# daac-tools/daachorse

Hardware: NVIDIA H100
Metric: input GB/s scanned, find_overlapping_iter, 675k-pat bytewise (higher is better)
Workload: dtype u8

## Files before the change

daachorse_b200/csrc/dev_image.cpp:

```cpp
#include "dev_image.h"

#include <algorithm>

namespace dach {

namespace {

bool fail_chains_terminate(const dach_pma* p, bool dead_is_terminal) {
    const size_t n = p->slots();
    std::vector<uint8_t> color(n, 0);
    std::vector<uint32_t> path;
    for (size_t start = 0; start < n; ++start) {
        if (color[start]) continue;
        path.clear();
        uint32_t s = uint32_t(start);
        for (;;) {
            if (s == kRoot || (dead_is_terminal && s == kDead) || color[s] == 2) break;
            if (color[s] == 1) return false;
            color[s] = 1;
            path.push_back(s);
            s = p->fail[s];
        }
        for (uint32_t v : path) color[v] = 2;
    }
// ... 148 lines not shown
            used[found ^ c] = 1;
            R->new_of_old[b_old ^ c] = found ^ c;
            moved[b_old ^ c] = 1;
            --n_free;
        }
    }
    for (size_t s = 0; s < n; ++s) {
        if (s != kRoot && s != kDead && !moved[s]) R->new_of_old[s] = uint32_t(s) + H;
        if (!rebased[s] && p->base[s] != 0) R->new_base[s] = p->base[s] + H;
    }
    R->vacant_check.assign(H, 0);
    for (uint32_t blk = 0; blk < H; blk += 256) {
        uint32_t ub = blk == 0 ? 0u : kNone;
        for (uint32_t b = blk; ub == kNone && b < blk + 256; ++b)
            if (!base_used[b]) {
                ub = b;
                break;
            }
        for (uint32_t v = blk; v < blk + 256; ++v)
            if (!used[v] || v == kRoot || v == kDead) R->vacant_check[v] = ub == kNone ? 0x100u : (0x100u | ((ub ^ v) & 0xffu));
    }
    R->hot_slots = H;
}

}

int build_image(const dach_pma* p, HostImage* img) {
    const size_t n = p->slots();
    const bool lm = is_leftmost(p->match_kind);
    img->charwise = p->charwise;
    img->match_kind = p->match_kind;
    img->n_slots = uint32_t(n);
    img->root_opos = n ? p->state_output_pos(kRoot) : 0;
    img->max_pattern_len = 0;
    for (const OutputRec& o : p->outputs)
        if (o.length > img->max_pattern_len) img->max_pattern_len = o.length;

    if (n >= 0x80000000ull) {
        set_error("automaton too large for the device image (2^31 slots)");
        return DACH_AUTOMATON_SCALE;
    }
    if (!fail_chains_terminate(p, p->charwise || lm)) {
        set_error("invalid automaton: a failure chain never reaches the root");
        return DACH_INVALID_AUTOMATON;
    }

    img->outputs.resize(p->outputs.size() * 4);
    for (size_t i = 0; i < p->outputs.size(); ++i) {
        img->outputs[i * 4 + 0] = p->outputs[i].value;
        img->outputs[i * 4 + 1] = p->outputs[i].length;
        img->outputs[i * 4 + 2] = p->outputs[i].parent;
        const uint32_t par = p->outputs[i].parent;
        img->outputs[i * 4 + 3] = 1u + (par ? img->outputs[(size_t)(par - 1) * 4 + 3] : 0u);
    }

    img->rec.resize(n * 4);
    if (!p->charwise) {
        auto skip_leaves = [&](uint32_t f) {
            while (f != kRoot && !(lm && f == kDead) && p->base[f] == 0) f = p->fail[f];
            return f;
        };
        for (size_t s = 0; s < n; ++s) {
            const uint32_t f = skip_leaves(p->fail[s]);
            const bool terminal = f == kRoot || (lm && f == kDead);
            uint32_t* r = &img->rec[s * 4];
            r[0] = p->base[s];
            r[1] = f;
            r[2] = terminal ? 0 : p->base[f];
            if (!terminal && !lm && skip_leaves(p->fail[f]) == kRoot) r[2] |= 0x80000000u;
            r[3] = p->opos_ch[s];
        }
        img->root_table.assign(256, kRoot);
        if (n && p->base[kRoot] != 0) {
            const uint32_t b = p->base[kRoot];
            for (uint32_t c = 0; c < 256; ++c) {
                const uint32_t ci = b ^ c;
                if (ci < n && (p->opos_ch[ci] & 0xff) == c) img->root_table[c] = ci;
            }
        }
        img->root_base = n ? p->base[kRoot] : 0;
        img->hot_slots = 0;
        if (n <= (size_t(1) << 24) && p->outputs.size() < (size_t(1) << 24)) {
            Relayout R;
            relayout_bytewise(p, img->want_hot_slots, &R);
            img->segmentable = R.textbook && R.max_depth <= img->max_pattern_len;
            const uint32_t H = R.hot_slots;
            const size_t N = n + H;
            img->hot_slots = H;
            img->n_cslots = uint32_t(N);
            img->crec.assign(N * 4, 0);
            img->opos_tab.assign(N, 0);
            img->new_of_old = R.new_of_old;
            img->old_of_new.assign(N, kRoot);
            img->root_base = n ? R.new_base[kRoot] : 0;
            auto nid = [&](uint32_t s) { return s < n ? R.new_of_old[s] : s; };
            for (size_t s = 0; s < n; ++s) {
                const uint32_t* w = &img->rec[s * 4];
                const uint32_t ns = R.new_of_old[s];
                img->old_of_new[ns] = uint32_t(s);
                uint32_t* r = &img->crec[size_t(ns) * 4];
                const uint32_t opos = p->opos_ch[s] >> 8;
                const uint32_t f = w[1];
                const bool terminal = f == kRoot || (lm && f == kDead);
                uint32_t flags = opos ? 1u : 0u;
                uint32_t fbase = terminal ? 0u : R.new_base[f];
                if (!lm) {
// ... 71 lines not shown
```

daachorse_b200/csrc/dev_image.h:

```cpp
#pragma once

#include <cstdint>
#include <vector>

#include "host.h"

namespace dach {

struct HostImage {
    bool charwise = false;
    uint8_t match_kind = 0;
    uint32_t n_slots = 0;
    uint32_t root_opos = 0;
    uint32_t max_pattern_len = 0;
    std::vector<uint32_t> rec;
    std::vector<uint32_t> outputs;
    std::vector<uint32_t> root_table;
    std::vector<uint32_t> crec;
    std::vector<uint32_t> opos_tab;
    uint32_t root_base = 0;
    uint32_t want_hot_slots = 65536;
    uint32_t hot_slots = 0;
    uint32_t n_cslots = 0;
    std::vector<uint32_t> new_of_old;
    std::vector<uint32_t> old_of_new;
    std::vector<uint32_t> mapper;
    bool segmentable = false;
};

int build_image(const dach_pma* p, HostImage* img);

}
```

daachorse_b200/csrc/dev_scan.cu:

```cuda
#include <cuda_runtime.h>

#include <unistd.h>

#include <algorithm>
#include <atomic>
#include <chrono>
#include <cstdio>
#include <cstdlib>
#include <cstring>
#include <memory>
#include <mutex>
#include <string>
#include <vector>

#include "dev_image.h"
#include "host.h"
#include "scan_lane.cuh"

namespace dach {


constexpr int kMaxThreads = 1024;
constexpr int kMaxDevices = 64;
constexpr uint32_t kRootBytes = 1024;
// ... 502 lines not shown
                                                 const uint4* outputs, const uint32_t* opos_tab) {
    if (ctrl->overflow) return;
    const unsigned long long b0m = base ? *base : 0ull;
    if (b0m + item_offs[n_items] > out_cap) return;
    out_words += b0m * 3ull;
    if (pad_like) out_words += (*pad_like * 3ull) & 3ull;
    const uint32_t used = min(ctrl->blk_cursor, pool_blocks);
    const uint32_t lane = threadIdx.x & 31;
    const uint64_t warp = (uint64_t)blockIdx.x * (blockDim.x >> 5) + (threadIdx.x >> 5);
    const uint64_t n_warps = (uint64_t)gridDim.x * (blockDim.x >> 5);
    for (uint64_t b0 = warp * U; b0 < used; b0 += n_warps * U) {
        uint4 h[U], o[U];
        uint2 ev[U];
        uint32_t len[U];
#pragma unroll
        for (int u = 0; u < U; ++u) {
            const uint64_t b = b0 + u < used ? b0 + u : b0;
            const uint32_t* blk = pool + (blkmap ? (uint64_t)blkmap[b] : b) * BLK_WORDS;
            h[u] = *reinterpret_cast<const uint4*>(blk);
            ev[u] = lane < BLK_EVENTS ? reinterpret_cast<const uint2*>(blk + BLK_HDR_WORDS)[lane] : make_uint2(0u, 0u);
        }
#pragma unroll
        for (int u = 0; u < U; ++u) {
            const uint32_t nev = min(BLK_EVENTS, ev_counts[h[u].x] - h[u].y * BLK_EVENTS);
            const bool on = b0 + u < used && lane < nev;
            const uint32_t op = on ? ld_u32(opos_tab + (ev[u].y & QSLOT_MASK)) : 0u;
            o[u] = on ? ld_u4(outputs + (op - 1)) : make_uint4(0u, 0u, 0u, 0u);
            len[u] = on ? (OVERLAP ? o[u].w : 1u) : 0u;
        }
#pragma unroll
        for (int u = 0; u < U; ++u) {
            uint32_t inc = len[u];
#pragma unroll
            for (int d = 1; d < 32; d <<= 1) {
                const uint32_t t = __shfl_up_sync(0xffffffffu, inc, d);
                if (lane >= (uint32_t)d) inc += t;
            }
            if (!len[u]) continue;
            uint32_t* dst = out_words + (item_offs[h[u].x] + h[u].z + (inc - len[u])) * 3ull;
            const uint32_t end = ev[u].x;
            uint4 r = o[u];
            for (uint32_t k = 0;;) {
                dst[0] = end - r.y;
                dst[1] = end;
                dst[2] = r.x;
                if (++k == len[u]) break;
                dst += 3;
                r = ld_u4(outputs + (r.z - 1));
            }
        }
    }
}

__global__ void __launch_bounds__(128, 10) k_push(const uint32_t* src, const unsigned long long* total_ptr, const unsigned long long* base,
                                               unsigned long long out_cap, const ScanCtrl* ctrl, uint32_t* out_words) {
    if (ctrl->overflow) return;
    const unsigned long long b0 = base ? *base : 0ull, total = *total_ptr;
    if (b0 + total > out_cap) return;
    uint32_t* dst = out_words + b0 * 3ull;
    src += (b0 * 3ull) & 3ull;
    const unsigned long long n_words = total * 3ull;
    const unsigned long long head = min((unsigned long long)((4u - (uint32_t)(((uintptr_t)dst >> 2) & 3u)) & 3u), n_words);
    const unsigned long long n_vec = (n_words - head) / 4ull;
    const unsigned long long tid = (unsigned long long)blockIdx.x * blockDim.x + threadIdx.x;
    const unsigned long long nth = (unsigned long long)gridDim.x * blockDim.x;
    const uint4* s4 = reinterpret_cast<const uint4*>(src + head);
    uint4* d4 = reinterpret_cast<uint4*>(dst + head);
    unsigned long long v = tid;
#pragma unroll 1
    for (; v + 3ull * nth < n_vec; v += 4ull * nth) {
        const uint4 a = s4[v], b = s4[v + nth], c = s4[v + 2ull * nth], e = s4[v + 3ull * nth];
        d4[v] = a;
        d4[v + nth] = b;
        d4[v + 2ull * nth] = c;
        d4[v + 3ull * nth] = e;
    }
#pragma unroll 1
    for (; v < n_vec; v += nth) d4[v] = s4[v];
    const unsigned long long tail0 = head + 4ull * n_vec;
    if (tid < head) dst[tid] = src[tid];
    if (tid < n_words - tail0) dst[tail0 + tid] = src[tail0 + tid];
}

__global__ void __launch_bounds__(256) k_final_offsets(const unsigned long long* seg_first, const unsigned long long* item_offs,
                                                        uint64_t n, const unsigned long long* base, int last,
                                                        unsigned long long* out_offs, const ScanCtrl* ctrl) {
    if (ctrl->bad_offsets) return;
    const uint64_t h = (uint64_t)blockIdx.x * blockDim.x + threadIdx.x;
    if (h < n || (h == n && last)) out_offs[h] = (base ? *base : 0ull) + item_offs[seg_first ? seg_first[h] : h];
}

__global__ void __launch_bounds__(256) k_add_base(const ScanCtrl* ctrl, const unsigned long long* out_offs, uint64_t n,
                                                   unsigned long long out_cap, const uint32_t* pos_in, uint32_t* out_words) {
    if (ctrl->overflow || ctrl->bad_offsets) return;
    const unsigned long long total = out_offs[n];
    if (total > out_cap) return;
    for (unsigned long long m = (unsigned long long)blockIdx.x * blockDim.x + threadIdx.x; m < total;
         m += (unsigned long long)gridDim.x * blockDim.x) {
        uint64_t lo = 0, hi = n;
        while (lo + 1 < hi) {
            const uint64_t mid = (lo + hi) / 2;
            if (out_offs[mid] <= m)
                lo = mid;
            else
                hi = mid;
        }
// ... 231 lines not shown
        red_add_u64(df_acc + (uint32_t)keys.keys[keys.list[i]], 1);
}

__global__ void __launch_bounds__(256) k_df_clear(DfSet a, DfSet b) {
    const unsigned int na = *a.n, nb = *b.n;
    for (unsigned int i = blockIdx.x * blockDim.x + threadIdx.x; i < na; i += gridDim.x * blockDim.x) a.keys[a.list[i]] = DF_EMPTY;
    for (unsigned int i = blockIdx.x * blockDim.x + threadIdx.x; i < nb; i += gridDim.x * blockDim.x) b.keys[b.list[i]] = DF_EMPTY;
}

__global__ void __launch_bounds__(256) k_df_commit(const unsigned long long* acc, unsigned long long* df, uint64_t n) {
    for (uint64_t i = blockIdx.x * (uint64_t)blockDim.x + threadIdx.x; i < n; i += (uint64_t)gridDim.x * blockDim.x) df[i] += acc[i];
}

}


using namespace dach;

namespace {

struct DevBuf {
    void* p = nullptr;
    size_t bytes = 0;
};

bool cuda_ok(cudaError_t e, const char* what) {
    if (e == cudaSuccess) return true;
    set_error(std::string(what) + ": " + cudaGetErrorString(e));
    return false;
}

bool ensure(DevBuf& b, size_t bytes) {
    if (b.bytes >= bytes && b.p) return true;
    if (b.p) cudaFree(b.p);
    b.p = nullptr;
    b.bytes = 0;
    const size_t want = std::max<size_t>(bytes, 256);
    if (!cuda_ok(cudaMalloc(&b.p, want), "cudaMalloc")) return false;
    b.bytes = want;
    return true;
}

struct HostPinned {
    unsigned long long total;
    ScanCtrl ctrl;
    unsigned long long tail_offs[2];
    unsigned long long total_rk;
};

struct Workspace {
    DevBuf counts, ev_counts, tiles, ctrl, pool;
    DevBuf nseg, seg_first, item_hay, item_beg, item_offs, n_items_dev;
    DevBuf blk_first, blkmap, tiles2;
    DevBuf stage;
    DevBuf items_rk, total_rk;
    DevBuf slot_hist, rec_hist, hist_acc;
    HostPinned* pinned = nullptr;
    cudaEvent_t ev[4] = {nullptr, nullptr, nullptr, nullptr};
    cudaEvent_t ev_scanned = nullptr, ev_placed = nullptr;
    cudaEvent_t ev_push[2] = {nullptr, nullptr};
    uint64_t job_n = 0, job_items = 0;
    uint32_t job_pool_blocks = 0;
    uint64_t job_cap = 0;
    bool job_seg = false, job_ordered = false, job_open = false, job_placed = false;
    bool job_events = false;
    bool refused = false;
    int job_mode = 0;
    cudaStream_t job_stream = nullptr;
    DevBuf text, offs, out, out_offs;
    void* offs_stage = nullptr;
    size_t offs_stage_bytes = 0;
    cudaStream_t stream = nullptr;
    bool init(bool with_stream) {
        if (!pinned && !cuda_ok(cudaMallocHost(reinterpret_cast<void**>(&pinned), sizeof(HostPinned)), "cudaMallocHost"))
            return false;
        for (int i = 0; i < 4; ++i)
            if (!ev[i] && !cuda_ok(cudaEventCreate(&ev[i]), "cudaEventCreate")) return false;
        if (!ev_scanned && !cuda_ok(cudaEventCreateWithFlags(&ev_scanned, cudaEventDisableTiming), "cudaEventCreate")) return false;
        if (!ev_placed && !cuda_ok(cudaEventCreateWithFlags(&ev_placed, cudaEventDisableTiming), "cudaEventCreate")) return false;
        for (int i = 0; i < 2; ++i)
            if (!ev_push[i] && !cuda_ok(cudaEventCreate(&ev_push[i]), "cudaEventCreate")) return false;
        if (with_stream && !stream && !cuda_ok(cudaStreamCreateWithFlags(&stream, cudaStreamNonBlocking), "cudaStreamCreate"))
            return false;
        return true;
    }
    void release() {
        for (DevBuf* b : {&counts, &ev_counts, &tiles, &ctrl, &pool, &text, &offs, &out, &out_offs, &nseg, &seg_first, &item_hay, &item_beg,
                          &item_offs, &n_items_dev, &blk_first, &blkmap, &tiles2, &stage, &items_rk, &total_rk, &slot_hist, &rec_hist,
                          &hist_acc})
            if (b->p) {
                cudaFree(b->p);
                b->p = nullptr;
                b->bytes = 0;
            }
        if (pinned) cudaFreeHost(pinned);
        pinned = nullptr;
        if (offs_stage) cudaFreeHost(offs_stage);
        offs_stage = nullptr;
        offs_stage_bytes = 0;
        for (int i = 0; i < 4; ++i)
            if (ev[i]) {
                cudaEventDestroy(ev[i]);
                ev[i] = nullptr;
            }
        for (int i = 0; i < 2; ++i)
            if (ev_push[i]) {
                cudaEventDestroy(ev_push[i]);
                ev_push[i] = nullptr;
            }
        if (ev_scanned) cudaEventDestroy(ev_scanned);
        if (ev_placed) cudaEventDestroy(ev_placed);
        ev_scanned = ev_placed = nullptr;
        if (stream) cudaStreamDestroy(stream);
        stream = nullptr;
    }
};

}

struct dach_dev {
    int device = 0;
    bool charwise = false;
    uint8_t match_kind = 0;
    uint32_t n_slots = 0, root_opos = 0, mapper_len = 0, max_pattern_len = 0;
    bool segmentable = false;
    uint32_t n_outputs = 0, max_value = 0, n_cslots = 0;
    size_t image_bytes = 0;
    int sm_count = 0;
    size_t smem_optin = 0;
    uint4* d_rec = nullptr;
    uint4* d_outputs = nullptr;
    uint32_t* d_root = nullptr;
    uint4* d_crec = nullptr;
    uint32_t* d_opos = nullptr;
    uint32_t* d_id_in = nullptr;
    uint32_t* d_id_out = nullptr;
    uint32_t hot_slots = 0;
    uint32_t root_base = 0;
    uint32_t* d_mapper = nullptr;
    void* image_base = nullptr;
    size_t image_alloc = 0;
    std::mutex mu;
    Workspace ws;
    static constexpr int kSlots = 4;
    Workspace slot[kSlots];
    int64_t opt_slice_mib = 64;
    int64_t opt_hot_entries = kHotAuto;
    int64_t opt_event_queue = 0;
    int64_t opt_hist_smem = 1024;
    int64_t opt_df_pairs = kDefaultDfPairs;
    int64_t opt_slice_ramp = 1;
    int64_t opt_tail_seg = 0;
    int64_t opt_gather_ordered = 1;
    int64_t opt_gather_u = 4;
    int64_t opt_reserve_sms = 0;
    int64_t opt_smem_pad_kib = 0;
    int64_t opt_seg_len = 0;
    int64_t opt_hot_records = 0;
    int64_t opt_threads = 1024;
    int64_t opt_ctas_per_sm = 1;
    int64_t opt_l2_hints = 2;
    int64_t opt_kernel = 3;
    std::atomic<uint64_t> launches{0};
    cudaEvent_t ev_ref = nullptr;
    double last_scan_ms = 0, last_total_ms = 0;
    uint64_t last_h2d = 0, last_d2h = 0;
    DevBuf df_tab[2], df_list[2], df_n, df_acc;
    uint32_t df_mask = 0, df_limit = 0;
    bool df_clean = false;
    uint64_t last_df_windows = 0, last_df_rescans = 0;
    std::atomic<int> refs{1};
};

struct dach_job {
    dach_dev* d = nullptr;
    Workspace W;
    uint64_t out_cap = ~0ull;
};

namespace {

struct DeviceGuard {
    int prev = -1;
    bool ok = false;
    explicit DeviceGuard(int dev) {
        if (cudaGetDevice(&prev) != cudaSuccess) prev = -1;
        ok = cuda_ok(cudaSetDevice(dev), "cudaSetDevice");
        if (!ok) cudaGetLastError();
    }
    ~DeviceGuard() {
        if (prev >= 0) cudaSetDevice(prev);
    }
};

template <bool CW, int MODE>
cudaError_t launch_scan_t(const ScanParams& P, int grid, int threads, size_t smem, cudaStream_t st) {
    static bool attr_done[kMaxDevices] = {};
    int dev = 0;
    cudaGetDevice(&dev);
    if (dev < 0 || dev >= kMaxDevices || !attr_done[dev]) {
        cudaError_t e = cudaFuncSetAttribute(k_scan<CW, MODE>, cudaFuncAttributeMaxDynamicSharedMemorySize, 226 * 1024);
// ... 275 lines not shown
            want &= ~uint64_t(255);
        }
        smem = (size_t)want * 16 + queues;
        if (d->opt_smem_pad_kib > 0) smem = std::min<size_t>(smem + ((size_t)d->opt_smem_pad_kib << 10), smem_budget);
        P.hot_n = 0;
        P.hot_entries = (uint32_t)want;
    } else {
        uint64_t hot = smem_budget > kRootBytes ? (smem_budget - kRootBytes) / 16 : 0;
        if (d->opt_hot_records >= 0) hot = std::min<uint64_t>(hot, (uint64_t)d->opt_hot_records);
        hot = std::min<uint64_t>(hot, d->n_slots);
        P.hot_n = (uint32_t)hot;
        smem = kRootBytes + (size_t)hot * 16;
    }
    return smem;
}

void enqueue_seg_table(dach_dev* d, Workspace& W, const uint64_t* d_offs, uint64_t n, uint32_t seg_len, uint32_t seg_from,
                       ScanParams& P, cudaStream_t st) {
    unsigned long long* tiles = static_cast<unsigned long long*>(W.tiles.p);
    unsigned long long* seg_first = static_cast<unsigned long long*>(W.seg_first.p);
    const unsigned hb = (unsigned)((n + 255) / 256), hb1 = (unsigned)((n + 1 + 255) / 256);
    const uint64_t nt = (n + kScanTile - 1) / kScanTile;
    uint32_t* nseg = static_cast<uint32_t*>(W.nseg.p);
    k_seg_count<<<hb, 256, 0, st>>>(d_offs, n, seg_len, seg_from, nseg, P.ctrl);
    k_offsets_tile_sums<1><<<(unsigned)nt, kScanThreads, 0, st>>>(nseg, n, tiles);
    k_offsets_scan_tiles<<<1, kScanThreads, 0, st>>>(tiles, nt);
    k_offsets_apply<1><<<(unsigned)nt, kScanThreads, 0, st>>>(nseg, n, tiles, seg_first);
    k_seg_fill<<<hb1, 256, 0, st>>>(seg_first, nseg, n, seg_len, static_cast<uint32_t*>(W.item_hay.p),
                                    static_cast<uint32_t*>(W.item_beg.p), static_cast<unsigned long long*>(W.n_items_dev.p));
    d->launches += 5;
    P.item_hay = static_cast<const uint32_t*>(W.item_hay.p);
    P.item_beg = static_cast<const uint32_t*>(W.item_beg.p);
    P.n_items_dev = static_cast<const unsigned long long*>(W.n_items_dev.p);
    P.seg_len = seg_len;
    P.seg_from = seg_from;
    P.warm = d->max_pattern_len ? d->max_pattern_len - 1 : 0;
}

int enqueue_scan(dach_dev* d, Workspace& W, int mode, const uint8_t* d_text, const uint8_t* text_lo, const uint8_t* text_end,
                 uint64_t text_bytes, const uint64_t* d_offs, uint64_t n, uint64_t cap_matches, cudaStream_t st,
                 uint32_t* d_state_io = nullptr) {
    W.refused = false;
    if (n > 0xfffffff0ull) {
        set_error("too many haystacks in one batch (max 2^32-16)");
        return DACH_INVALID_ARGUMENT;
    }
    if (W.job_open) cudaStreamWaitEvent(st, W.ev_placed, 0);
    W.job_n = n;
    W.job_cap = cap_matches;
    W.job_items = n;
    W.job_seg = false;
    W.job_ordered = false;
    W.job_events = false;
    W.job_stream = st;
    W.job_open = true;
    if (!ensure(W.ctrl, sizeof(ScanCtrl)) || !ensure(W.item_offs, 16)) return DACH_CUDA_ERROR;
    if (!cuda_ok(cudaMemsetAsync(W.ctrl.p, 0, sizeof(ScanCtrl), st), "memset ctrl")) return DACH_CUDA_ERROR;
    cudaEventRecord(W.ev[0], st);
    cudaEventRecord(W.ev[3], st);
    if (n == 0) {
        cudaMemsetAsync(W.item_offs.p, 0, 8, st);
        cudaEventRecord(W.ev[1], st);
        cudaEventRecord(W.ev_scanned, st);
        return DACH_OK;
    }
    int threads = (int)std::min<int64_t>(std::max<int64_t>(d->opt_threads, 32), kMaxThreads);
    threads = (threads / 32) * 32;
    int ctas_per_sm = (int)std::min<int64_t>(std::max<int64_t>(d->opt_ctas_per_sm, 1), 2048 / threads);
    const int free_sms = (int)std::min<int64_t>(std::max<int64_t>(d->opt_reserve_sms, 0), d->sm_count - 1);
    const int grid = (d->sm_count - free_sms) * ctas_per_sm;
    const bool v1 = d->opt_kernel >= 1 && d->d_crec && !(mode == M_FIND && d->root_opos != 0);
    const bool cw_machine = v1 && d->charwise;
    const bool lm_machine = v1 && !d->charwise && mode == M_LEFTMOST;
    const bool std2 = v1 && !d->charwise && mode != M_LEFTMOST && d->opt_kernel >= 2 && d->root_base != 0;
    const bool std3 = std2 && d->opt_kernel >= 3;
    const bool duo = std3 && d->opt_kernel >= 4 && ctas_per_sm == 1;
    const bool events = std3 && !duo;
    const bool direct = events && ctas_per_sm == 1 && d->opt_event_queue == 0;

    if (d_state_io && !std2 && !cw_machine) {
        set_error("stream chunks need a Standard lane machine (find / find_overlapping, at most 2^24 states, bytewise: "
                  "BASE(ROOT) != 0, no empty pattern for find)");
        return DACH_INVALID_ARGUMENT;
    }

    bool seg = v1 && !d->charwise && !d_state_io && (mode == M_OVERLAPPING || mode == M_NO_SUFFIX) && d->opt_seg_len >= 0 && d->segmentable;
    uint32_t seg_len = 0, seg_from = 0;
    uint64_t n_items_max = n;
    if (seg) {
        const uint64_t lanes = (uint64_t)grid * threads;
        const uint64_t warm = d->max_pattern_len ? d->max_pattern_len - 1 : 0;
        const uint64_t floor_len = std::max<uint64_t>(256, 8 * warm);
        uint64_t want;
        uint64_t tail_bytes = text_bytes;
        if (d->opt_seg_len > 0) {
            want = (uint64_t)d->opt_seg_len;
        } else if (d->opt_tail_seg && n >= 4 * lanes && n < 0xffffffffull) {
            const uint64_t n_tail = 2 * lanes;
            seg_from = (uint32_t)(n - n_tail);
            want = std::max(text_bytes / n / 8 + 1, floor_len);
            cudaMemcpyAsync(&W.pinned->tail_offs[0], d_offs + seg_from, 8, cudaMemcpyDeviceToHost, st);
            cudaMemcpyAsync(&W.pinned->tail_offs[1], d_offs + n, 8, cudaMemcpyDeviceToHost, st);
            if (!cuda_ok(cudaStreamSynchronize(st), "read tail size")) return DACH_CUDA_ERROR;
            tail_bytes = W.pinned->tail_offs[1] - W.pinned->tail_offs[0];
        } else {
            want = std::max(text_bytes / (2 * lanes) + 1, floor_len);
// ... 2 lines not shown
        if (want >= text_bytes || want >= (1ull << 31)) {
            seg = false;
        } else {
            seg_len = (uint32_t)want;
            n_items_max = n + tail_bytes / seg_len + 1;
            if (n_items_max > 0xfffffff0ull) seg = false, n_items_max = n;
        }
    }
    const uint64_t n_tiles = (n_items_max + kScanTile - 1) / kScanTile;
    uint64_t pool_blocks64 = cap_matches / BLK_MATCHES + n_items_max + 1024;
    if (pool_blocks64 > 0xffffff00ull) pool_blocks64 = 0xffffff00ull;
    const uint32_t pool_blocks = (uint32_t)pool_blocks64;
    if (!ensure(W.counts, n_items_max * 4) || !ensure(W.tiles, n_tiles * 8) || !ensure(W.item_offs, (n_items_max + 1) * 8) ||
        !ensure(W.pool, (size_t)pool_blocks * BLK_WORDS * 4) || (events && !ensure(W.ev_counts, n_items_max * 4)))
        return DACH_CUDA_ERROR;
    if (seg && (!ensure(W.nseg, n * 4) || !ensure(W.seg_first, (n + 1) * 8) || !ensure(W.item_hay, n_items_max * 4) ||
                !ensure(W.item_beg, n_items_max * 4) || !ensure(W.n_items_dev, 8)))
        return DACH_CUDA_ERROR;

    ScanParams P = image_params(d, d_text, text_lo, text_end, d_offs, n);
    P.counts = static_cast<uint32_t*>(W.counts.p);
    P.ev_counts = events ? static_cast<uint32_t*>(W.ev_counts.p) : nullptr;
    P.pool = static_cast<uint32_t*>(W.pool.p);
    P.pool_blocks = pool_blocks;
    P.ctrl = static_cast<ScanCtrl*>(W.ctrl.p);
    P.state_io = d_state_io;
    const size_t smem = plan_smem(d, P, v1, std3, threads, ctas_per_sm, duo ? 2 : direct ? 0 : 1);

    unsigned long long* tiles = static_cast<unsigned long long*>(W.tiles.p);
    unsigned long long* item_offs = static_cast<unsigned long long*>(W.item_offs.p);
    k_check_offsets<<<(unsigned)((n + 255) / 256), 256, 0, st>>>(d_offs, n, (uint64_t)(text_end - d_text), P.ctrl);
    ++d->launches;
    if (seg) {
        cudaMemsetAsync(W.counts.p, 0, n_items_max * 4, st);
        if (events) cudaMemsetAsync(W.ev_counts.p, 0, n_items_max * 4, st);
        enqueue_seg_table(d, W, d_offs, n, seg_len, seg_from, P, st);
    }
    cudaEventRecord(W.ev[3], st);
    if (!cuda_ok(cw_machine   ? launch_cw(mode, P, grid, std::min(threads, 1024), smem, st)
                 : lm_machine ? launch_lm(P, grid, std::min(threads, 1024), smem, st)
                 : duo        ? launch_duo(mode, P, grid, threads, smem, st)
                 : direct     ? launch_direct(mode, P, grid, threads, smem, st)
                 : v1        ? launch_std(std3 ? 3 : std2 ? 2 : 1, mode, P, grid, threads, smem, st,
                                           ctas_per_sm >= 2 && threads <= 768 && grid % 2 == 0)
                              : launch_scan(d->charwise, mode, P, grid, threads, smem, st),
                 "k_scan launch"))
        return DACH_CUDA_ERROR;
    cudaEventRecord(W.ev[1], st);
    k_offsets_tile_sums<1><<<(unsigned)n_tiles, kScanThreads, 0, st>>>(P.counts, n_items_max, tiles);
    k_offsets_scan_tiles<<<1, kScanThreads, 0, st>>>(tiles, n_tiles);
    k_offsets_apply<1><<<(unsigned)n_tiles, kScanThreads, 0, st>>>(P.counts, n_items_max, tiles, item_offs);
    d->launches += 4;
    const bool ordered = d->opt_gather_ordered >= 2 || (d->opt_gather_ordered == 1 && text_bytes >= (256ull << 20));
    if (ordered) {
        if (!ensure(W.blk_first, (n_items_max + 1) * 8) || !ensure(W.blkmap, (size_t)pool_blocks * 4) || !ensure(W.tiles2, n_tiles * 8))
            return DACH_CUDA_ERROR;
        unsigned long long* tiles2 = static_cast<unsigned long long*>(W.tiles2.p);
        unsigned long long* blk_first = static_cast<unsigned long long*>(W.blk_first.p);
        if (events) {
            k_offsets_tile_sums<BLK_EVENTS><<<(unsigned)n_tiles, kScanThreads, 0, st>>>(P.ev_counts, n_items_max, tiles2);
            k_offsets_scan_tiles<<<1, kScanThreads, 0, st>>>(tiles2, n_tiles);
            k_offsets_apply<BLK_EVENTS><<<(unsigned)n_tiles, kScanThreads, 0, st>>>(P.ev_counts, n_items_max, tiles2, blk_first);
        } else {
            k_offsets_tile_sums<BLK_MATCHES><<<(unsigned)n_tiles, kScanThreads, 0, st>>>(P.counts, n_items_max, tiles2);
            k_offsets_scan_tiles<<<1, kScanThreads, 0, st>>>(tiles2, n_tiles);
            k_offsets_apply<BLK_MATCHES><<<(unsigned)n_tiles, kScanThreads, 0, st>>>(P.counts, n_items_max, tiles2, blk_first);
        }
        k_blk_index<<<d->sm_count * 8, 256, 0, st>>>(P.pool, P.ctrl, pool_blocks, blk_first, static_cast<uint32_t*>(W.blkmap.p));
        d->launches += 4;
    }
    if (!cuda_ok(cudaGetLastError(), "kernel launch")) return DACH_CUDA_ERROR;
    cudaEventRecord(W.ev_scanned, st);
    W.job_items = n_items_max;
    W.job_seg = seg;
    W.job_ordered = ordered;
    W.job_events = events;
    W.job_mode = mode;
    W.job_pool_blocks = pool_blocks;
    return DACH_OK;
}

int enqueue_place(dach_dev* d, Workspace& W, dach_match* d_out, uint64_t out_cap, uint64_t* d_out_offs,
                  const unsigned long long* d_base, bool last, cudaStream_t st, const uint32_t* d_pos_in = nullptr,
                  bool staged = false, bool dma = false, uint64_t h_base = 0, uint64_t h_total = 0) {
    if (!W.job_open) {
        set_error("no scan to place");
        return DACH_INVALID_ARGUMENT;
    }
    if (st != W.job_stream) cudaStreamWaitEvent(st, W.ev_scanned, 0);
    const uint64_t n = W.job_n, n_items = W.job_items;
    const ScanCtrl* ctrl = static_cast<const ScanCtrl*>(W.ctrl.p);
    const unsigned long long* item_offs = static_cast<const unsigned long long*>(W.item_offs.p);
    unsigned long long* offs64 = reinterpret_cast<unsigned long long*>(d_out_offs);
    const int gather_grid = d->sm_count * 8;
    if (n) {
        const uint32_t* pool = static_cast<const uint32_t*>(W.pool.p);
        const uint32_t* counts = static_cast<const uint32_t*>(W.counts.p);
        const uint32_t* blkmap = W.job_ordered ? static_cast<const uint32_t*>(W.blkmap.p) : nullptr;
        uint32_t* out_words = reinterpret_cast<uint32_t*>(d_out);
        const unsigned long long* g_base = d_base;
        unsigned long long g_cap = out_cap;
        if (staged) {
            if (!ensure(W.stage, W.job_cap * sizeof(dach_match) + 256)) return DACH_CUDA_ERROR;
            out_words = static_cast<uint32_t*>(W.stage.p);
            g_base = nullptr;
            g_cap = W.job_cap;
        }
        const unsigned long long* pad_like = staged ? d_base : nullptr;
        if (W.job_events) {
            const uint32_t* ev_counts = static_cast<const uint32_t*>(W.ev_counts.p);
            if (W.job_mode == M_OVERLAPPING)
                k_expand<true, 2><<<gather_grid, 256, 0, st>>>(pool, ctrl, W.job_pool_blocks, ev_counts, item_offs, n_items, g_cap, g_base,
                                                                out_words, blkmap, pad_like, d->d_outputs, d->d_opos);
            else
                k_expand<false, 2><<<gather_grid, 256, 0, st>>>(pool, ctrl, W.job_pool_blocks, ev_counts, item_offs, n_items, g_cap, g_base,
                                                                 out_words, blkmap, pad_like, d->d_outputs, d->d_opos);
        } else if (d->opt_gather_u >= 8)
            k_gather<8><<<gather_grid, 256, 0, st>>>(pool, ctrl, W.job_pool_blocks, counts, item_offs, n_items, g_cap, g_base, out_words, blkmap, pad_like);
        else if (d->opt_gather_u <= 2)
            k_gather<2><<<gather_grid, 256, 0, st>>>(pool, ctrl, W.job_pool_blocks, counts, item_offs, n_items, g_cap, g_base, out_words, blkmap, pad_like);
        else
            k_gather<4><<<gather_grid, 256, 0, st>>>(pool, ctrl, W.job_pool_blocks, counts, item_offs, n_items, g_cap, g_base, out_words, blkmap, pad_like);
        ++d->launches;
        if (staged) {
            cudaEventRecord(W.ev_push[0], st);
            if (dma) {
                if (h_total && h_base + h_total <= out_cap &&
                    !cuda_ok(cudaMemcpyAsync(reinterpret_cast<uint32_t*>(d_out) + h_base * 3ull, out_words + ((h_base * 3ull) & 3ull),
                                             h_total * sizeof(dach_match), cudaMemcpyDefault, st),
                             "peer copy"))
                    return DACH_CUDA_ERROR;
            } else {
                k_push<<<d->sm_count * 4, 128, 0, st>>>(out_words, item_offs + n_items, d_base, out_cap, ctrl, reinterpret_cast<uint32_t*>(d_out));
                ++d->launches;
            }
            cudaEventRecord(W.ev_push[1], st);
        }
    }
    k_final_offsets<<<(unsigned)((n + 1 + 255) / 256), 256, 0, st>>>(
        W.job_seg ? static_cast<const unsigned long long*>(W.seg_first.p) : nullptr, item_offs, n, d_base, last ? 1 : 0, offs64, ctrl);
    ++d->launches;
    if (d_pos_in && n) {
        k_add_base<<<gather_grid, 256, 0, st>>>(ctrl, offs64, n, out_cap, d_pos_in, reinterpret_cast<uint32_t*>(d_out));
        ++d->launches;
    }
    if (!cuda_ok(cudaGetLastError(), "kernel launch")) return DACH_CUDA_ERROR;
    cudaEventRecord(W.ev[2], st);
    cudaMemcpyAsync(&W.pinned->total, item_offs + n_items, 8, cudaMemcpyDeviceToHost, st);
    cudaMemcpyAsync(&W.pinned->ctrl, W.ctrl.p, sizeof(ScanCtrl), cudaMemcpyDeviceToHost, st);
    cudaEventRecord(W.ev_placed, st);
    W.job_placed = true;
    return DACH_OK;
}

int finish_scan(dach_dev* d, Workspace& W, uint64_t out_cap, uint64_t* needed) {
    W.refused = false;
    if (!cuda_ok(cudaEventSynchronize(W.ev_placed), "scan pipeline")) return DACH_CUDA_ERROR;
    float ms = 0;
    if (cudaEventElapsedTime(&ms, W.ev[3], W.ev[1]) == cudaSuccess) d->last_scan_ms = ms;
    if (cudaEventElapsedTime(&ms, W.ev[0], W.ev[2]) == cudaSuccess) d->last_total_ms = ms;
    const uint64_t total = W.pinned->total + ((uint64_t)W.pinned->ctrl.carries << 32);
    if (needed) *needed = total;
// ... 674 lines not shown
        return f();
    } catch (const std::bad_alloc&) {
        set_error("out of memory");
        return DACH_AUTOMATON_SCALE;
    } catch (const std::exception& e) {
        set_error(std::string("internal error: ") + e.what());
        return DACH_INVALID_ARGUMENT;
    } catch (...) {
        set_error("internal error");
        return DACH_INVALID_ARGUMENT;
    }
}

}

extern "C" {

int dach_dev_upload(const dach_pma* pma, int device, dach_dev** out) {
    if (!out) return DACH_INVALID_ARGUMENT;
    *out = nullptr;
    if (!pma) {
        set_error("null automaton");
        return DACH_INVALID_ARGUMENT;
    }
    return guarded([&]() -> int {
        HostImage img;
        if (const char* e = getenv("DACH_HOT_SLOTS")) img.want_hot_slots = (uint32_t)strtoul(e, nullptr, 10);
        const int rc = build_image(pma, &img);
        if (rc) return rc;
        int ndev = 0;
        if (!cuda_ok(cudaGetDeviceCount(&ndev), "cudaGetDeviceCount")) return DACH_CUDA_ERROR;
        if (device < 0 || device >= ndev) {
            set_error("no such CUDA device");
            return DACH_CUDA_ERROR;
        }
        DeviceGuard g(device);
        if (!g.ok) return DACH_CUDA_ERROR;
        std::unique_ptr<dach_dev> d(new dach_dev());
        d->device = device;
        d->charwise = img.charwise;
        d->match_kind = img.match_kind;
        d->n_slots = img.n_slots;
        d->root_opos = img.root_opos;
        d->max_pattern_len = img.max_pattern_len;
        d->segmentable = img.segmentable;
        d->mapper_len = (uint32_t)img.mapper.size();
        d->n_outputs = (uint32_t)(img.outputs.size() / 4);
        for (uint32_t i = 0; i < d->n_outputs; ++i) d->max_value = std::max(d->max_value, img.outputs[(size_t)i * 4]);
        d->n_cslots = (uint32_t)img.opos_tab.size();
        cudaDeviceProp prop;
        if (!cuda_ok(cudaGetDeviceProperties(&prop, device), "cudaGetDeviceProperties")) return DACH_CUDA_ERROR;
        d->sm_count = prop.multiProcessorCount;
        d->smem_optin = prop.sharedMemPerBlockOptin;
        constexpr int kParts = 8;
        const std::vector<uint32_t>* parts[kParts] = {&img.rec, &img.outputs, &img.root_table, &img.mapper, &img.crec, &img.opos_tab,
                                                       &img.new_of_old, &img.old_of_new};
        size_t part_off[kParts], total = 0;
        for (int i = 0; i < kParts; ++i) {
            part_off[i] = total;
            total += (std::max<size_t>(parts[i]->size() * 4, 16) + 511) & ~size_t(511);
            d->image_bytes += parts[i]->size() * 4;
        }
        bool ok = cuda_ok(cudaMalloc(&d->image_base, total), "cudaMalloc image");
        d->image_alloc = total;
        for (int i = 0; ok && i < kParts; ++i)
            if (!parts[i]->empty())
                ok = cuda_ok(cudaMemcpy(static_cast<char*>(d->image_base) + part_off[i], parts[i]->data(), parts[i]->size() * 4,
                                        cudaMemcpyHostToDevice),
                             "upload image");
        if (ok) {
            char* b = static_cast<char*>(d->image_base);
            d->d_rec = reinterpret_cast<uint4*>(b + part_off[0]);
            d->d_outputs = reinterpret_cast<uint4*>(b + part_off[1]);
            d->d_root = reinterpret_cast<uint32_t*>(b + part_off[2]);
            d->d_mapper = reinterpret_cast<uint32_t*>(b + part_off[3]);
            if (!img.crec.empty()) {
                d->d_crec = reinterpret_cast<uint4*>(b + part_off[4]);
                d->d_opos = reinterpret_cast<uint32_t*>(b + part_off[5]);
                if (img.hot_slots) {
                    d->d_id_in = reinterpret_cast<uint32_t*>(b + part_off[6]);
                    d->d_id_out = reinterpret_cast<uint32_t*>(b + part_off[7]);
                }
                d->hot_slots = img.hot_slots;
            }
            d->root_base = img.root_base;
        }
        ok = ok && install_policies((int)d->opt_l2_hints) && d->ws.init(false);
        if (!ok) {
            dach_dev_free(d.release());
            return DACH_CUDA_ERROR;
        }
        *out = d.release();
        return DACH_OK;
    });
}

void dach_dev_free(dach_dev* d) {
    if (!d || --d->refs > 0) return;
    DeviceGuard g(d->device);
    cudaFree(d->image_base);
    if (d->ev_ref) cudaEventDestroy(d->ev_ref);
    d->ws.release();
    for (Workspace& w : d->slot) w.release();
    for (DevBuf* b : {&d->df_tab[0], &d->df_tab[1], &d->df_list[0], &d->df_list[1], &d->df_n, &d->df_acc})
        if (b->p) cudaFree(b->p);
    delete d;
}

size_t dach_dev_image_bytes(const dach_dev* d) { return d ? d->image_bytes : 0; }

int dach_dev_scan_batch(dach_dev* d, int mode, const uint8_t* d_text, const uint64_t* d_offs, uint64_t n,
                        uint64_t text_bytes, dach_match* d_out, uint64_t out_cap, uint64_t* d_out_offs,
                        uint64_t* needed, void* stream) {
    if (!d || !d_offs || !d_out_offs || (out_cap && !d_out)) {
        set_error("null argument");
        return DACH_INVALID_ARGUMENT;
    }
    const int rc = check_mode(d, mode);
    if (rc) return rc;
    return guarded([&]() -> int {
        std::lock_guard<std::mutex> lk(d->mu);
        DeviceGuard g(d->device);
        if (!g.ok) return DACH_CUDA_ERROR;
        return scan_locked(d, d->ws, mode, d_text, d_text, d_text + text_bytes, text_bytes, d_offs, n, d_out, out_cap, d_out_offs, needed,
                           static_cast<cudaStream_t>(stream));
    });
// ... 511 lines not shown
void dach_group_free(dach_group* G) {
    if (!G) return;
    DeviceGuard g(G->device);
    cudaDeviceSynchronize();
    for (int i = 0; i < G->n_ipc; ++i) cudaIpcCloseMemHandle(G->ipc_opened[i]);
    if (G->rank == 0) {
        cudaFree(G->out);
        cudaFree(G->offs);
    }
    cudaFree(G->ctl);
    if (G->pinned) cudaFreeHost(G->pinned);
    if (G->h_vals) cudaFreeHost(G->h_vals);
    delete G;
}

uint64_t dach_dev_kernel_launches(const dach_dev* d) { return d ? d->launches.load() : 0; }
double dach_dev_last_scan_kernel_ms(const dach_dev* d) { return d ? d->last_scan_ms : 0; }
double dach_dev_last_total_ms(const dach_dev* d) { return d ? d->last_total_ms : 0; }
uint64_t dach_dev_last_h2d_bytes(const dach_dev* d) { return d ? d->last_h2d : 0; }
uint64_t dach_dev_last_d2h_bytes(const dach_dev* d) { return d ? d->last_d2h : 0; }

int dach_dev_set_option(dach_dev* d, const char* name, int64_t value) {
    if (!d || !name) return DACH_INVALID_ARGUMENT;
    std::lock_guard<std::mutex> lk(d->mu);
    const std::string k(name);
    if (k == "hot_records")
        d->opt_hot_records = value;
    else if (k == "threads")
        d->opt_threads = value;
    else if (k == "ctas_per_sm")
        d->opt_ctas_per_sm = value;
    else if (k == "kernel")
        d->opt_kernel = value;
    else if (k == "slice_mib")
        d->opt_slice_mib = value;
    else if (k == "seg_len")
        d->opt_seg_len = value;
    else if (k == "slice_ramp")
        d->opt_slice_ramp = value;
    else if (k == "tail_seg")
        d->opt_tail_seg = value;
    else if (k == "gather_ordered")
        d->opt_gather_ordered = value;
    else if (k == "gather_u")
        d->opt_gather_u = value;
    else if (k == "reserve_sms")
        d->opt_reserve_sms = value;
    else if (k == "smem_pad_kib")
        d->opt_smem_pad_kib = value;
    else if (k == "hot_entries")
        d->opt_hot_entries = value;
    else if (k == "event_queue")
        d->opt_event_queue = value;
    else if (k == "hist_smem")
        d->opt_hist_smem = value;
    else if (k == "df_pairs")
        d->opt_df_pairs = value;
    else if (k == "l2_hints") {
        d->opt_l2_hints = value;
        DeviceGuard g(d->device);
        if (!g.ok || !install_policies((int)value)) return DACH_CUDA_ERROR;
    } else {
        set_error("unknown option " + k);
        return DACH_INVALID_ARGUMENT;
    }
    return DACH_OK;
}

}
```

Baseline: 129.5.

## Precompute block descriptors and packed output pairs for ordered event expansion

Adds a per-block descriptor pass that resolves each pool block's output offset and event count once. The output image gains a packed 'pairs' table that stores a match and its parent inline, plus a chain-length class. The new expand kernel uses the table to write one- or two-output chains without walking the output linked list, and falls back to the full walk only for longer chains. The aim is fewer dependent global loads in the gather stage, at the cost of extra image memory and a descriptor buffer. It only takes effect in ordered gather mode with events enabled.

```diff
diff --git a/daachorse_b200/csrc/dev_image.cpp b/daachorse_b200/csrc/dev_image.cpp
--- a/daachorse_b200/csrc/dev_image.cpp
+++ b/daachorse_b200/csrc/dev_image.cpp
@@ -224,6 +224,17 @@
         img->outputs[i * 4 + 2] = p->outputs[i].parent;
         const uint32_t par = p->outputs[i].parent;
         img->outputs[i * 4 + 3] = 1u + (par ? img->outputs[(size_t)(par - 1) * 4 + 3] : 0u);
+    }
+    img->pairs.clear();
+    if (img->max_pattern_len < PAIR_LEN_MASK) {
+        img->pairs.resize(p->outputs.size() * 4);
+        for (size_t i = 0; i < p->outputs.size(); ++i) {
+            const uint32_t par = p->outputs[i].parent, len = img->outputs[i * 4 + 3];
+            img->pairs[i * 4 + 0] = p->outputs[i].value;
+            img->pairs[i * 4 + 1] = p->outputs[i].length;
+            img->pairs[i * 4 + 2] = par ? p->outputs[par - 1].value : 0u;
+            img->pairs[i * 4 + 3] = (par ? p->outputs[par - 1].length : 0u) | (len < 3u ? len : 3u) << PAIR_CLASS_SHIFT;
+        }
     }
 
     img->rec.resize(n * 4);
diff --git a/daachorse_b200/csrc/dev_image.h b/daachorse_b200/csrc/dev_image.h
--- a/daachorse_b200/csrc/dev_image.h
+++ b/daachorse_b200/csrc/dev_image.h
@@ -7,6 +7,9 @@
 
 namespace dach {
 
+constexpr uint32_t PAIR_CLASS_SHIFT = 30;
+constexpr uint32_t PAIR_LEN_MASK = (1u << PAIR_CLASS_SHIFT) - 1u;
+
 struct HostImage {
     bool charwise = false;
     uint8_t match_kind = 0;
@@ -15,6 +18,7 @@
     uint32_t max_pattern_len = 0;
     std::vector<uint32_t> rec;
     std::vector<uint32_t> outputs;
+    std::vector<uint32_t> pairs;
     std::vector<uint32_t> root_table;
     std::vector<uint32_t> crec;
     std::vector<uint32_t> opos_tab;
diff --git a/daachorse_b200/csrc/dev_scan.cu b/daachorse_b200/csrc/dev_scan.cu
--- a/daachorse_b200/csrc/dev_scan.cu
+++ b/daachorse_b200/csrc/dev_scan.cu
@@ -578,6 +578,92 @@
     }
 }
 
+__global__ void __launch_bounds__(256) k_blk_desc(const uint32_t* pool, const ScanCtrl* ctrl, uint32_t pool_blocks,
+                                                   const unsigned long long* blk_first, const uint32_t* ev_counts,
+                                                   const unsigned long long* item_offs, uint4* desc) {
+    if (ctrl->overflow) return;
+    const uint32_t used = min(ctrl->blk_cursor, pool_blocks);
+    for (uint64_t b = (uint64_t)blockIdx.x * blockDim.x + threadIdx.x; b < used; b += (uint64_t)gridDim.x * blockDim.x) {
+        const uint4 h = *reinterpret_cast<const uint4*>(pool + b * BLK_WORDS);
+        const unsigned long long j = blk_first[h.x] + h.y;
+        if (j < used) {
+            const unsigned long long at = item_offs[h.x] + h.z;
+            desc[j] = make_uint4((uint32_t)b, min(BLK_EVENTS, ev_counts[h.x] - h.y * BLK_EVENTS), (uint32_t)at, (uint32_t)(at >> 32));
+        }
+    }
+}
+
+constexpr uint32_t EXP_THREADS = 256;
+template <bool OVERLAP, int U>
+__global__ void __launch_bounds__(EXP_THREADS) k_expand_desc(const uint32_t* pool, const ScanCtrl* ctrl, uint32_t pool_blocks,
+                                                            const uint4* desc, const unsigned long long* item_offs,
+                                                            uint64_t n_items, unsigned long long out_cap, const unsigned long long* base,
+                                                            uint32_t* out_words, const unsigned long long* pad_like,
+                                                            const uint4* pairs, const uint4* outputs, const uint32_t* opos_tab) {
+    if (ctrl->overflow) return;
+    const unsigned long long b0m = base ? *base : 0ull;
+    if (b0m + item_offs[n_items] > out_cap) return;
+    out_words += b0m * 3ull;
+    if (pad_like) out_words += (*pad_like * 3ull) & 3ull;
+    const uint32_t used = min(ctrl->blk_cursor, pool_blocks);
+    const uint32_t lane = threadIdx.x & 31;
+    const uint64_t warp = (uint64_t)blockIdx.x * (blockDim.x >> 5) + (threadIdx.x >> 5);
+    const uint64_t n_warps = (uint64_t)gridDim.x * (blockDim.x >> 5);
+    for (uint64_t b0 = warp * U; b0 < used; b0 += n_warps * U) {
+        uint4 dsc[U], p[U];
+        uint2 ev[U];
+#pragma unroll
+        for (int u = 0; u < U; ++u) {
+            dsc[u] = desc[b0 + u < used ? b0 + u : b0];
+            if (b0 + u >= used) dsc[u].y = 0;
+        }
+#pragma unroll
+        for (int u = 0; u < U; ++u)
+            ev[u] = lane < dsc[u].y ? reinterpret_cast<const uint2*>(pool + (uint64_t)dsc[u].x * BLK_WORDS + BLK_HDR_WORDS)[lane]
+                                    : make_uint2(0u, 0u);
+        uint32_t op[U];
+#pragma unroll
+        for (int u = 0; u < U; ++u) op[u] = lane < dsc[u].y ? ld_u32(opos_tab + (ev[u].y & QSLOT_MASK)) : 0u;
+#pragma unroll
+        for (int u = 0; u < U; ++u) p[u] = op[u] ? ld_u4(pairs + (op[u] - 1)) : make_uint4(0u, 0u, 0u, 0u);
+#pragma unroll
+        for (int u = 0; u < U; ++u) {
+            if (!dsc[u].y) continue;
+            const uint32_t cls = OVERLAP ? p[u].w >> PAIR_CLASS_SHIFT : (op[u] ? 1u : 0u);
+            uint4 r = make_uint4(0u, 0u, 0u, 0u);
+            if (cls == 3u) r = ld_u4(outputs + (op[u] - 1));
+            const uint32_t len = cls == 3u ? r.w : cls;
+            uint32_t inc = len;
+#pragma unroll
+            for (int d = 1; d < 32; d <<= 1) {
+                const uint32_t t = __shfl_up_sync(0xffffffffu, inc, d);
+                if (lane >= (uint32_t)d) inc += t;
+            }
+            uint32_t* w = out_words + (((unsigned long long)dsc[u].w << 32 | dsc[u].z) + (inc - len)) * 3ull;
+            const uint32_t end = ev[u].x;
+            if (cls == 1u || cls == 2u) {
+                w[0] = end - p[u].y;
+                w[1] = end;
+                w[2] = p[u].x;
+                if (cls == 2u) {
+                    w[3] = end - (p[u].w & PAIR_LEN_MASK);
+                    w[4] = end;
+                    w[5] = p[u].z;
+                }
+            } else if (cls == 3u) {
+                for (uint32_t k = 0;;) {
+                    w[0] = end - r.y;
+                    w[1] = end;
+                    w[2] = r.x;
+                    if (++k == len) break;
+                    w += 3;
+                    r = ld_u4(outputs + (r.z - 1));
+                }
+            }
+        }
+    }
+}
+
 __global__ void __launch_bounds__(128, 10) k_push(const uint32_t* src, const unsigned long long* total_ptr, const unsigned long long* base,
                                                unsigned long long out_cap, const ScanCtrl* ctrl, uint32_t* out_words) {
     if (ctrl->overflow) return;
@@ -915,6 +1001,7 @@
     DevBuf counts, ev_counts, tiles, ctrl, pool;
     DevBuf nseg, seg_first, item_hay, item_beg, item_offs, n_items_dev;
     DevBuf blk_first, blkmap, tiles2;
+    DevBuf desc;
     DevBuf stage;
     DevBuf items_rk, total_rk;
     DevBuf slot_hist, rec_hist, hist_acc;
@@ -927,6 +1014,7 @@
     uint64_t job_cap = 0;
     bool job_seg = false, job_ordered = false, job_open = false, job_placed = false;
     bool job_events = false;
+    bool job_desc = false;
     bool refused = false;
     int job_mode = 0;
     cudaStream_t job_stream = nullptr;
@@ -949,7 +1037,7 @@
     }
     void release() {
         for (DevBuf* b : {&counts, &ev_counts, &tiles, &ctrl, &pool, &text, &offs, &out, &out_offs, &nseg, &seg_first, &item_hay, &item_beg,
-                          &item_offs, &n_items_dev, &blk_first, &blkmap, &tiles2, &stage, &items_rk, &total_rk, &slot_hist, &rec_hist,
+                          &item_offs, &n_items_dev, &blk_first, &blkmap, &desc, &tiles2, &stage, &items_rk, &total_rk, &slot_hist, &rec_hist,
                           &hist_acc})
             if (b->p) {
                 cudaFree(b->p);
@@ -996,6 +1084,7 @@
     uint32_t* d_root = nullptr;
     uint4* d_crec = nullptr;
     uint32_t* d_opos = nullptr;
+    uint4* d_pairs = nullptr;
     uint32_t* d_id_in = nullptr;
     uint32_t* d_id_out = nullptr;
     uint32_t hot_slots = 0;
@@ -1010,6 +1099,8 @@
     int64_t opt_slice_mib = 64;
     int64_t opt_hot_entries = kHotAuto;
     int64_t opt_event_queue = 0;
+    int64_t opt_expand_desc = 1;
+    int64_t opt_expand_u = 2;
     int64_t opt_hist_smem = 1024;
     int64_t opt_df_pairs = kDefaultDfPairs;
     int64_t opt_slice_ramp = 1;
@@ -1391,6 +1482,7 @@
     W.job_seg = false;
     W.job_ordered = false;
     W.job_events = false;
+    W.job_desc = false;
     W.job_stream = st;
     W.job_open = true;
     if (!ensure(W.ctrl, sizeof(ScanCtrl)) || !ensure(W.item_offs, 16)) return DACH_CUDA_ERROR;
@@ -1499,8 +1591,10 @@
     k_offsets_apply<1><<<(unsigned)n_tiles, kScanThreads, 0, st>>>(P.counts, n_items_max, tiles, item_offs);
     d->launches += 4;
     const bool ordered = d->opt_gather_ordered >= 2 || (d->opt_gather_ordered == 1 && text_bytes >= (256ull << 20));
+    const bool use_desc = ordered && events && d->d_pairs && d->opt_expand_desc != 0;
     if (ordered) {
-        if (!ensure(W.blk_first, (n_items_max + 1) * 8) || !ensure(W.blkmap, (size_t)pool_blocks * 4) || !ensure(W.tiles2, n_tiles * 8))
+        if (!ensure(W.blk_first, (n_items_max + 1) * 8) || !ensure(W.tiles2, n_tiles * 8) ||
+            !(use_desc ? ensure(W.desc, (size_t)pool_blocks * 16) : ensure(W.blkmap, (size_t)pool_blocks * 4)))
             return DACH_CUDA_ERROR;
         unsigned long long* tiles2 = static_cast<unsigned long long*>(W.tiles2.p);
         unsigned long long* blk_first = static_cast<unsigned long long*>(W.blk_first.p);
@@ -1513,7 +1607,11 @@
             k_offsets_scan_tiles<<<1, kScanThreads, 0, st>>>(tiles2, n_tiles);
             k_offsets_apply<BLK_MATCHES><<<(unsigned)n_tiles, kScanThreads, 0, st>>>(P.counts, n_items_max, tiles2, blk_first);
         }
-        k_blk_index<<<d->sm_count * 8, 256, 0, st>>>(P.pool, P.ctrl, pool_blocks, blk_first, static_cast<uint32_t*>(W.blkmap.p));
+        if (use_desc)
+            k_blk_desc<<<d->sm_count * 8, 256, 0, st>>>(P.pool, P.ctrl, pool_blocks, blk_first, P.ev_counts, item_offs,
+                                                        static_cast<uint4*>(W.desc.p));
+        else
+            k_blk_index<<<d->sm_count * 8, 256, 0, st>>>(P.pool, P.ctrl, pool_blocks, blk_first, static_cast<uint32_t*>(W.blkmap.p));
         d->launches += 4;
     }
     if (!cuda_ok(cudaGetLastError(), "kernel launch")) return DACH_CUDA_ERROR;
@@ -1522,6 +1620,7 @@
     W.job_seg = seg;
     W.job_ordered = ordered;
     W.job_events = events;
+    W.job_desc = use_desc;
     W.job_mode = mode;
     W.job_pool_blocks = pool_blocks;
     return DACH_OK;
@@ -1554,7 +1653,15 @@
             g_cap = W.job_cap;
         }
         const unsigned long long* pad_like = staged ? d_base : nullptr;
-        if (W.job_events) {
+        if (W.job_desc) {
+            const uint4* desc = static_cast<const uint4*>(W.desc.p);
+            const int u = d->opt_expand_u >= 8 ? 8 : d->opt_expand_u <= 2 ? 2 : 4;
+            const bool ov = W.job_mode == M_OVERLAPPING;
+            auto kern = ov ? (u == 8 ? k_expand_desc<true, 8> : u == 2 ? k_expand_desc<true, 2> : k_expand_desc<true, 4>)
+                           : (u == 8 ? k_expand_desc<false, 8> : u == 2 ? k_expand_desc<false, 2> : k_expand_desc<false, 4>);
+            kern<<<gather_grid, EXP_THREADS, 0, st>>>(pool, ctrl, W.job_pool_blocks, desc, item_offs, n_items, g_cap, g_base, out_words,
+                                                      pad_like, d->d_pairs, d->d_outputs, d->d_opos);
+        } else if (W.job_events) {
             const uint32_t* ev_counts = static_cast<const uint32_t*>(W.ev_counts.p);
             if (W.job_mode == M_OVERLAPPING)
                 k_expand<true, 2><<<gather_grid, 256, 0, st>>>(pool, ctrl, W.job_pool_blocks, ev_counts, item_offs, n_items, g_cap, g_base,
@@ -2335,9 +2442,9 @@
         if (!cuda_ok(cudaGetDeviceProperties(&prop, device), "cudaGetDeviceProperties")) return DACH_CUDA_ERROR;
         d->sm_count = prop.multiProcessorCount;
         d->smem_optin = prop.sharedMemPerBlockOptin;
-        constexpr int kParts = 8;
+        constexpr int kParts = 9;
         const std::vector<uint32_t>* parts[kParts] = {&img.rec, &img.outputs, &img.root_table, &img.mapper, &img.crec, &img.opos_tab,
-                                                       &img.new_of_old, &img.old_of_new};
+                                                       &img.new_of_old, &img.old_of_new, &img.pairs};
         size_t part_off[kParts], total = 0;
         for (int i = 0; i < kParts; ++i) {
             part_off[i] = total;
@@ -2355,6 +2462,7 @@
             char* b = static_cast<char*>(d->image_base);
             d->d_rec = reinterpret_cast<uint4*>(b + part_off[0]);
             d->d_outputs = reinterpret_cast<uint4*>(b + part_off[1]);
+            if (!img.pairs.empty()) d->d_pairs = reinterpret_cast<uint4*>(b + part_off[8]);
             d->d_root = reinterpret_cast<uint32_t*>(b + part_off[2]);
             d->d_mapper = reinterpret_cast<uint32_t*>(b + part_off[3]);
             if (!img.crec.empty()) {
@@ -2972,6 +3080,10 @@
         d->opt_hot_entries = value;
     else if (k == "event_queue")
         d->opt_event_queue = value;
+    else if (k == "expand_desc")
+        d->opt_expand_desc = value;
+    else if (k == "expand_u")
+        d->opt_expand_u = value;
     else if (k == "hist_smem")
         d->opt_hist_smem = value;
     else if (k == "df_pairs")
```

After: 133.7, median of 6. 1.03x the previous value.
